# F-Fer/SLAM-Loop-Closing

Measured on AMD Instinct MI355X. Metric: Hamming distances/sec (256-bit ORB) for all-vs-all loop search, 1/2/4/8 GPUs, higher is better.
Workload: dtype u32

## Files before the change

include/lcm.h:

```cpp
#ifndef LCM_H_
#define LCM_H_

#include <stddef.h>
#include <stdint.h>

#ifdef __cplusplus
extern "C" {
#endif

#if defined(__GNUC__)
#define LCM_API __attribute__((visibility("default")))
#else
#define LCM_API
#endif

#define LCM_DESC_BYTES 32
#define LCM_DESC_WORDS 8
#define LCM_MAX_TRAIN_ROWS (1 << 22)

typedef enum lcm_status {
    LCM_OK = 0,
    LCM_ERR_INVALID_ARG = -1,
    LCM_ERR_NO_DEVICE = -2,
    LCM_ERR_HIP = -3,
// ... 362 lines not shown
                                          const int* query_frame_ids, int n_queries, int* ticket);
LCM_API int  lcm_group_query_collect_batch(lcm_group* g, int ticket, lcm_score* out_scores, size_t cap, size_t* n_out,
                                           size_t* offsets);
LCM_API int  lcm_group_online_stats_read(lcm_group* g, lcm_online_stats* out, int reset);
LCM_API int  lcm_group_detect_loops(lcm_group* g, int current_frame_id, const uint8_t* query, int nq, int n_keypoints,
                                    lcm_loop_candidate* out, int cap, int* n_out);
LCM_API int  lcm_merge_shard_scores(const lcm_score* const* shard_scores, const size_t* shard_counts, int world,
                                    const int32_t* ids, int n_frames, int min_gap,
                                    lcm_score* out, size_t cap, size_t* n_out, size_t* offsets);

LCM_API int  lcm_merge_shard_scores_device(lcm_handle* h, const void* d_gathered, const size_t* shard_counts, int world,
                                           const int32_t* ids, int n_frames, int min_gap,
                                           void* d_merged, size_t cap, size_t* n_out);

typedef enum lcm_tuning { LCM_TUNE_ITEM_SLOTS = 0, LCM_TUNE_ONLINE_SPLIT = 1, LCM_TUNE_PACKED = 2, LCM_TUNE_ONLINE_STREAMS = 3,
                          LCM_TUNE_PACKED_SCRATCH_MB = 4, LCM_TUNE_PAIR_UPLOAD_KERNEL = 5, LCM_TUNE_PAIR_HOST_FOLD = 6 } lcm_tuning;
LCM_API int  lcm_set_tuning(lcm_handle* h, int knob, int value);

LCM_API int  lcm_dev_alloc(lcm_handle* h, size_t bytes, void** d_ptr);
LCM_API int  lcm_dev_free(lcm_handle* h, void* d_ptr);
LCM_API int  lcm_dev_upload(lcm_handle* h, void* d_dst, const void* src, size_t bytes);
LCM_API int  lcm_dev_download(lcm_handle* h, void* dst, const void* d_src, size_t bytes);

#ifdef __cplusplus
}
#endif
#endif
```

slam-loop-closing_amd/capi.py:

```python
from __future__ import annotations

import ctypes as C
import os
from typing import Optional, Sequence, Tuple

import numpy as np

_HERE = os.path.dirname(os.path.abspath(__file__))
LIB_PATH = os.environ.get("LCM_LIB_PATH") or os.path.join(_HERE, "lib", "liblcm_hip.so")
DESC_BYTES = 32
SIFT_BYTES = 128
KEY_SHIFT = 22
TUNE_ITEM_SLOTS, TUNE_ONLINE_SPLIT, TUNE_PACKED, TUNE_ONLINE_STREAMS, TUNE_PACKED_SCRATCH_MB = 0, 1, 2, 3, 4
TUNE_PAIR_UPLOAD_KERNEL, TUNE_PAIR_HOST_FOLD = 5, 6


OK, ERR_INVALID_ARG, ERR_NO_DEVICE, ERR_HIP, ERR_CAPACITY, ERR_ORDER, ERR_NOT_FOUND, ERR_OOM = 0, -1, -2, -3, -4, -5, -6, -7


class LcmError(RuntimeError):
    def __init__(self, code: int, msg: str):
        super().__init__(f"lcm error {code}: {msg}")
        self.code = code


class Params(C.Structure):
    _fields_ = [("ratio", C.c_int32), ("dist_floor", C.c_int32), ("min_matches", C.c_int32),
                ("min_gap", C.c_int32), ("sim_threshold", C.c_double), ("cross_check", C.c_int32),
                ("reserved", C.c_int32)]
# ... 1534 lines not shown
```

slam-loop-closing_amd/csrc/lcm_api.cpp:

```cpp
#include "lcm_internal.h"

namespace lcm {
std::string& last_error() { static thread_local std::string e; return e; }
int fail(int code, const char* fmt, ...) {
    char buf[512];
    va_list ap;
    va_start(ap, fmt);
    vsnprintf(buf, sizeof buf, fmt, ap);
    va_end(ap);
    last_error() = buf;
    return code;
}
void set_last_error(const char* msg) { last_error() = msg ? msg : ""; }
}

namespace lcm {

int set_device(const lcm_handle* h) {
    HIP_TRY(hipSetDevice(h->device));
    return LCM_OK;
}

int wait_db(lcm_handle* h) {
    if (h->pending_copy) {
// ... 261 lines not shown
            if (value < 0 || value > 64) return fail(LCM_ERR_INVALID_ARG, "item slots must be 0 (automatic) .. 64");
            h->tune_item_slots = value; h->plan.key = 0; return LCM_OK;
        case LCM_TUNE_ONLINE_SPLIT:
            if (value != -1 && value != 0 && value != 1 && value != 2 && value != 4 && value != 16 && value != 32)
                return fail(LCM_ERR_INVALID_ARG, "online split must be -1 (automatic), 0 (off), 1, 2, 4 (rows per lane of a 256-thread workgroup), 16 or 32 (64 / 128 threads x 8 rows)");
            h->tune_online_split = value; return LCM_OK;
        case LCM_TUNE_ONLINE_STREAMS:
            if (value != 0 && value != 1) return fail(LCM_ERR_INVALID_ARG, "online streams must be 0 (the handle's stream) or 1 (one per query slot)");
            h->tune_online_streams = value; return LCM_OK;
        case LCM_TUNE_PAIR_UPLOAD_KERNEL:
            if (value != 0 && value != 1) return fail(LCM_ERR_INVALID_ARG, "pair upload must be 0 (hipMemcpyAsync) or 1 (kernel)");
            h->tune_pair_upload_kernel = value; return LCM_OK;
        case LCM_TUNE_PAIR_HOST_FOLD:
            if (value != 0 && value != 1) return fail(LCM_ERR_INVALID_ARG, "pair host fold must be 0 (device buffer + copy) or 1 (pinned host memory)");
            h->tune_pair_host_fold = value; return LCM_OK;
        case LCM_TUNE_PACKED_SCRATCH_MB:
            if (value < 1 || value > 65536) return fail(LCM_ERR_INVALID_ARG, "packed scratch must be 1 .. 65536 MiB per chunk");
            h->pk_scratch_cfg_words = h->pk_scratch_words = (size_t)value << 18; h->plan.key = 0; return LCM_OK;
        case LCM_TUNE_PACKED:
            if (value < -1 || value > 2) return fail(LCM_ERR_INVALID_ARG, "packed rows must be -1 (automatic), 0 (off), 1 (on) or 2 (on, 1536-row columns)");
            h->tune_packed = value; h->plan.key = 0; return LCM_OK;
        default: return fail(LCM_ERR_INVALID_ARG, "unknown tuning knob %d", knob);
    }
}


static int db_reserve_impl(lcm_handle* h, int n_frames, int max_desc) {
    if (!h || n_frames < 0 || max_desc < 0) return fail(LCM_ERR_INVALID_ARG, "bad argument");
    if (max_desc > MAX_FRAME_ROWS) return fail(LCM_ERR_CAPACITY, "a stored frame may hold at most %d rows (got %d)", MAX_FRAME_ROWS, max_desc);
    int rc = set_device(h); if (rc) return rc;
// ... 173 lines not shown


int lcm_loop_test(const lcm_params* p, const lcm_score* s, int n_query_kp, int n_train_kp, double* similarity) {
    if (similarity) *similarity = 0.0;
    if (!p || !s) return 0;
    const int den = std::min(n_query_kp, n_train_kp);
    if (den <= 0) return 0;
    const double sim = (double)s->good_count / (double)den;
    if (similarity) *similarity = sim;
    return (sim > p->sim_threshold) && ((long long)s->good_count >= (long long)p->min_matches);
}

int lcm_last_launch_info(const lcm_handle* hc, lcm_launch_info* info) {
    lcm_handle* h = const_cast<lcm_handle*>(hc);
    if (!h || !info) return fail(LCM_ERR_INVALID_ARG, "NULL argument");
    if (h->info_pending || h->aux_pending) { const int rc = set_device(h); if (rc) return rc; }
    if (h->info_pending) {
        HIP_TRY(hipEventSynchronize(h->ev_stop));
        float ms = 0.f;
        HIP_TRY(hipEventElapsedTime(&ms, h->ev_start, h->ev_stop));
        h->info.kernel_ms = ms;
        h->info.aux_kernel_ms = 0.0;
        h->info_pending = false;
        h->info.score_launches = 0; h->info.score_ms_sum = 0.0;
        if (h->info.route == LCM_ROUTE_PACKED) {
            double fold = 0.0, score = 0.0;
            for (size_t k = 0; k + 3 <= h->fold_ev_used && k + 3 <= h->fold_ev.size(); k += 3) {
                float f = 0.f;
                if (hipEventElapsedTime(&f, h->fold_ev[k], h->fold_ev[k + 1]) == hipSuccess) score += f; else (void)hipGetLastError();
                if (hipEventElapsedTime(&f, h->fold_ev[k + 1], h->fold_ev[k + 2]) == hipSuccess) fold += f; else (void)hipGetLastError();
                ++h->info.score_launches;
// ... 79 lines not shown
```

slam-loop-closing_amd/csrc/lcm_internal.h:

```cpp
#pragma once
#include "../../include/lcm.h"

#include <hip/hip_runtime.h>
#include <sys/stat.h>

#include <algorithm>
#include <cstdarg>
#include <cstdio>
#include <cstdlib>
#include <cstring>
#include <new>
#include <string>
#include <vector>

#include "lcm_kernels.h"
#include "lcm_l2_host.h"
#include "lcm_verify_host.h"

namespace lcm {
std::string& last_error();
int fail(int code, const char* fmt, ...) __attribute__((format(printf, 2, 3)));
void set_last_error(const char* msg);
}

// ... 110 lines not shown
    hipStream_t copy_stream = nullptr;
    hipStream_t stream2 = nullptr;
    hipEvent_t ev_fork = nullptr, ev_join = nullptr;
    hipEvent_t db_ready = nullptr;
    hipEvent_t ev_start = nullptr, ev_stop = nullptr;
    hipEvent_t ev_aux_start = nullptr, ev_aux_stop = nullptr;
    bool aux_pending = false;
    std::vector<hipEvent_t> fold_ev;
    size_t fold_ev_used = 0;
    int variant = 0;
    int tune_item_slots = 0;
    int tune_online_split = -1;
    int tune_pair_upload_kernel = 1;
    int tune_pair_host_fold = 1;
    int tune_online_streams = 1;
    size_t pk_scratch_cfg_words = (size_t)1 << 28;
    size_t pk_scratch_words = (size_t)1 << 28;
    bool pk_oom_retry = false;
    int tune_packed = -1;

    uint8_t* d_rows = nullptr;
    int32_t* d_counts = nullptr;
    int cap_frames = 0;
    int stride_rows = 0;
    std::vector<FrameMeta> frames;
    bool pending_copy = false;
    bool db_ready_recorded = false;

    uint8_t* h_stage[lcm::STAGE_BUFS] = {nullptr, nullptr};
    size_t h_stage_bytes = 0;
// ... 65 lines not shown
    struct PoseScratch {
        double* d_E = nullptr;        size_t d_E_n = 0;
        uint8_t* d_mask_in = nullptr; size_t d_mask_in_n = 0;
        double* d_cand = nullptr;     size_t d_cand_n = 0;
        lcm_pose_result* d_res = nullptr; size_t d_res_n = 0;
        uint8_t* d_mask = nullptr;    size_t d_mask_n = 0;
    } pose;
    struct LoScratch {
        int32_t* d_seeds = nullptr;   size_t d_seeds_n = 0;
        lcm_lo_info* d_info = nullptr; size_t d_info_n = 0;
        double* d_models = nullptr;   size_t d_models_n = 0;
        int32_t* d_seam = nullptr;    size_t d_seam_n = 0;
    } lo;
    lcm_launch_info info{};
    bool info_pending = false;
};


namespace {

template <typename T>
int ensure_dev(T*& p, size_t& have, size_t need, size_t slack_bytes = 0) {
    if (need <= have && p) return LCM_OK;
    if (p) HIP_TRY(hipFree(p));
    p = nullptr; have = 0;
    size_t n = std::max<size_t>(need, 16);
    HIP_TRY(hipMalloc((void**)&p, n * sizeof(T) + slack_bytes));
    have = n;
    return LCM_OK;
}
// ... 153 lines not shown
```

slam-loop-closing_amd/csrc/lcm_kernels.h:

```cpp
#pragma once
#include <hip/hip_runtime.h>
#include <stdint.h>

namespace lcm {

constexpr int KEY_SHIFT = 22;
constexpr uint32_t KEY_IDX_MASK = (1u << KEY_SHIFT) - 1;
constexpr int MAX_FUSED_QUERY_ROWS = 2048;
constexpr int MAX_QUERY_BATCH = 16;

struct WorkItem {
    uint32_t q_frame;
    uint32_t slot_begin;
    uint32_t n_slots;
    uint32_t out_offset;
};

struct PairItem {
    uint32_t q_row;
    uint32_t t_row;
    uint32_t nq_nt;
    uint32_t out_offset;
};

// ... 2 lines not shown
    const int32_t*  q_counts;
    uint32_t        q_stride_words;
    const uint32_t* db_rows;
    const int32_t*  db_counts;
    uint32_t        db_stride_words;
    const WorkItem* items;
    const PairItem* pair_items;
    void*           scores;
    uint32_t*       keys;
    uint32_t        keys_stride;
    uint32_t*       idx_sums;
    int32_t         ratio;
    int32_t         dist_floor;
    uint32_t        imp_chunks, imp_chunk_rows, imp_spi, imp_total;
    int32_t         imp_nq;
    const uint32_t* pk_vstart;
    const uint32_t* pk_qframe;
    const uint32_t* pk_elig;
    const uint32_t* pk_pairs;
    uint32_t*       pk_dist;
    uint32_t        pk_n;
    uint32_t        pk_col_rows;
    uint32_t        pk_stride;
    uint32_t        pk_slot0;
    uint32_t        imp_nbatch;
    uint32_t        bat_wg[MAX_QUERY_BATCH + 1];
    uint32_t        bat_pair[MAX_QUERY_BATCH + 1];
    int32_t         bat_nq[MAX_QUERY_BATCH];
    uint32_t        bat_elig[MAX_QUERY_BATCH];
};

hipError_t launch_score(const ScoreArgs& a, uint32_t n_items, int max_query_rows, bool write_keys, int variant,
                        hipStream_t st);
hipError_t launch_score_packed(const ScoreArgs& a, uint32_t n_items, bool argmin, hipStream_t st);

hipError_t launch_score_split(const ScoreArgs& a, uint32_t n_items, int qpt, hipStream_t st);
struct FinalizeArgs {
    const uint32_t* dist;
    uint32_t        padded_rows;
    int32_t         nq;
    const int32_t*  db_counts;
    uint32_t        slot_begin;
    void*           scores;
    int32_t         ratio, dist_floor;
    uint32_t        n_batch;
    uint32_t        bat_pair[MAX_QUERY_BATCH + 1];
    int32_t         bat_nq[MAX_QUERY_BATCH];
};
hipError_t launch_finalize(const FinalizeArgs& a, uint32_t n_pairs, hipStream_t st);

struct PairDesc {
    uint32_t first_item;
    uint32_t n_seg;
    uint32_t seg_rows;
// ... 283 lines not shown
```

slam-loop-closing_amd/csrc/lcm_kernels.hip:

```cpp
#include <hip/hip_runtime.h>
#include <stdint.h>

#include <algorithm>
#include <atomic>

#include "lcm_kernels.h"

#ifndef LCM_INNER_PRIO
#define LCM_INNER_PRIO 1
#endif

namespace lcm {

typedef const uint32_t __attribute__((address_space(4))) * sptr_t;
typedef const int32_t __attribute__((address_space(4))) * siptr_t;

__device__ __forceinline__ void fold2(uint32_t& best, const uint32_t (&q)[8], const uint32_t* s, uint32_t t0, uint32_t t1) {
#if LCM_INNER_PRIO
    uint32_t d0, d1, x0, x1;
    asm volatile(
        "v_xor_b32_e32 %3, %5, %21\n\tv_xor_b32_e32 %4, %13, %21\n\ts_setprio 3\n\t"
        "v_bcnt_u32_b32 %1, %3, 0\n\tv_bcnt_u32_b32 %2, %4, 0\n\ts_setprio 0\n\t"
        "v_xor_b32_e32 %3, %6, %22\n\tv_xor_b32_e32 %4, %14, %22\n\ts_setprio 3\n\t"
        "v_bcnt_u32_b32 %1, %3, %1\n\tv_bcnt_u32_b32 %2, %4, %2\n\ts_setprio 0\n\t"
// ... 149 lines not shown
        pair_nt = (int)(pi.nq_nt >> 12);
        pair_t_row = pi.t_row;
        q_word0 = (size_t)pi.q_row * 8;
    } else if (a.items) {
        it = a.items[blockIdx.x];
        nq = a.q_counts[it.q_frame];
        q_word0 = (size_t)it.q_frame * a.q_stride_words;
    } else {
        uint32_t b = blockIdx.x, qi = 0, total = a.imp_total, pair0 = 0;
        int rows = a.imp_nq;
        if (a.imp_nbatch) {
            while (qi + 1 < a.imp_nbatch && b >= a.bat_wg[qi + 1]) ++qi;
            b -= a.bat_wg[qi];
            total = a.bat_elig[qi]; pair0 = a.bat_pair[qi]; rows = a.bat_nq[qi];
        }
        const uint32_t c = b % a.imp_chunks, g = b / a.imp_chunks;
        it.q_frame = qi * a.imp_chunks + c;
        it.slot_begin = g * a.imp_spi;
        it.n_slots = min(a.imp_spi, total - it.slot_begin);
        it.out_offset = (pair0 + it.slot_begin) * a.imp_chunks + c;
        nq = min((int)a.imp_chunk_rows, rows - (int)(c * a.imp_chunk_rows));
        q_word0 = (size_t)it.q_frame * a.q_stride_words;
    }

    uint32_t q[QPT][8];
    auto valid = [&](int j) { return j * THREADS + tid < nq; };
    if (PACKED) {
        {
            uint32_t c = it.out_offset;
            const uint32_t v0 = it.q_frame * (uint32_t)(THREADS * QPT);
#pragma unroll 1
            for (int j = 0; j < QPT; ++j) {
                const uint32_t v = v0 + (uint32_t)(j * THREADS + tid);
                uint32_t meta = 0xFFFFFFFFu;
                if (j * THREADS + tid < nq) {
                    while (a.pk_vstart[c + 1] <= v) ++c;
                    meta = c;
// ... 381 lines not shown
    return hipGetLastError();
}

__global__ __launch_bounds__(256) void k_finalize_pairs(FinalizeArgs a, uint32_t n_pairs) {
    const int lane = threadIdx.x & 63;
    const uint32_t pair = blockIdx.x * 4u + (threadIdx.x >> 6);
    if (pair >= n_pairs) return;
    int nq = a.nq;
    uint32_t slot = a.slot_begin + pair;
    if (a.n_batch) {
        uint32_t b = 0;
        while (b + 1 < a.n_batch && pair >= a.bat_pair[b + 1]) ++b;
        nq = a.bat_nq[b];
        slot = pair - a.bat_pair[b];
    }
    const uint4* d = reinterpret_cast<const uint4*>(a.dist + (size_t)pair * a.padded_rows);
    uint32_t v[32];
#pragma unroll
    for (int i = 0; i < 8; ++i) {
        const int r0 = (i * 64 + lane) * 4;
        uint4 x = make_uint4(0xFFFFFFFFu, 0xFFFFFFFFu, 0xFFFFFFFFu, 0xFFFFFFFFu);
        if (r0 < nq) x = d[i * 64 + lane];
        v[4 * i + 0] = x.x;
        v[4 * i + 1] = r0 + 1 < nq ? x.y : 0xFFFFFFFFu;
        v[4 * i + 2] = r0 + 2 < nq ? x.z : 0xFFFFFFFFu;
        v[4 * i + 3] = r0 + 3 < nq ? x.w : 0xFFFFFFFFu;
    }
    uint32_t dmin = 0xFFFFFFFFu;
#pragma unroll
    for (int k = 0; k < 32; ++k) dmin = min(dmin, v[k]);
#pragma unroll
    for (int o = 32; o >= 1; o >>= 1) dmin = min(dmin, (uint32_t)__shfl_xor((int)dmin, o, 64));
    const uint32_t thr = max((uint32_t)a.ratio * dmin, (uint32_t)a.dist_floor);
    uint32_t cnt = 0;
#pragma unroll
    for (int k = 0; k < 32; ++k) cnt += (v[k] != 0xFFFFFFFFu && v[k] <= thr) ? 1u : 0u;
#pragma unroll
    for (int o = 32; o >= 1; o >>= 1) cnt += (uint32_t)__shfl_xor((int)cnt, o, 64);
    if (lane == 0) {
        const int nt = a.db_counts[slot];
        const bool empty = (nq <= 0) || (nt <= 0) || dmin == 0xFFFFFFFFu;
// ... 308 lines not shown
```

slam-loop-closing_amd/csrc/lcm_online.cpp:

```cpp
#include "lcm_internal.h"

static inline bool is_split(int qpt) { return qpt == 1 || qpt == 2 || qpt == 4 || qpt == 16 || qpt == 32; }
static inline int split_chunk_rows(int qpt) { return qpt == 16 ? 512 : qpt == 32 ? 1024 : 256 * qpt; }

static int pick_online_split(const lcm_handle* h, int max_nq, size_t pairs, bool batch) {
    if (h->variant != 0 || max_nq <= 512) return 0;
    if (h->tune_online_split >= 0) return h->tune_online_split;
    if (batch) return pairs < lcm::ONLINE_SPLIT_MAX_PAIRS ? 2 : 0;
    return pairs < 48 ? 1 : pairs < 4096 ? 2 : 0;
}

extern "C" {

static void account_prefix(lcm_handle* h, int nq, int n_elig) {
    uint64_t dist = 0, bytes = (uint64_t)nq * 32;
    for (int s = 0; s < n_elig; ++s) { dist += (uint64_t)nq * h->frames[s].n; bytes += (uint64_t)h->frames[s].n * 32 + 8; }
    h->info.pairs = (uint64_t)n_elig; h->info.distances = dist; h->info.algo_bytes = bytes;
}

static int enqueue_query(lcm_handle* h, QuerySlot& q, const uint32_t* d_q, int nq, int n_elig, hipStream_t S) {
    q.n_elig = n_elig; q.nq = nq; q.n_batch = 0;
    q.acc_pairs = q.acc_distances = q.acc_bytes = 0; q.acc_launches = 0; q.acc_queries = 1;
    if (n_elig <= 0) { HIP_TRY(hipEventRecord(q.done, S)); return LCM_OK; }
    int rc = wait_db(h); if (rc) return rc;
    if (h->params.cross_check) {
        rc = ensure_dev(q.d_scores, q.d_scores_n, (size_t)n_elig); if (rc) return rc;
        rc = ensure_pinned(q.h_scores, q.h_scores_n, (size_t)n_elig); if (rc) return rc;
        const uint32_t row0 = 0;
        HIP_TRY(hipEventRecord(q.k0, h->stream));
        rc = cross_score_prefixes(h, (const uint8_t*)d_q, &row0, &nq, &n_elig, 1, q.d_scores, nullptr); if (rc) return rc;
        HIP_TRY(hipEventRecord(q.k1, h->stream));
        q.acc_pairs = h->info.pairs; q.acc_distances = h->info.distances; q.acc_bytes = h->info.algo_bytes; q.acc_launches = h->info.launches;
        HIP_TRY(hipMemcpyAsync(q.h_scores, q.d_scores, sizeof(lcm_score) * (size_t)n_elig, hipMemcpyDeviceToHost, h->stream));
        HIP_TRY(hipEventRecord(q.done, h->stream));
        return LCM_OK;
    }
    if (h->variant >= 4) {
        return mfma_online(h, q, d_q, std::max(nq, 1), 1, &nq, &n_elig);
    }
    const int qpt = pick_online_split(h, nq, (size_t)n_elig, false);
    rc = ensure_dev(q.d_scores, q.d_scores_n, (size_t)n_elig); if (rc) return rc;
    rc = ensure_pinned(q.h_scores, q.h_scores_n, (size_t)n_elig); if (rc) return rc;
    lcm::ScoreArgs a{};
    a.q_rows = d_q; a.q_counts = nullptr; a.items = nullptr;
    a.db_rows = (const uint32_t*)h->d_rows; a.db_counts = h->d_counts; a.db_stride_words = (uint32_t)h->stride_rows * LCM_DESC_WORDS;
    a.ratio = h->params.ratio; a.dist_floor = h->params.dist_floor;
    a.imp_nq = nq; a.imp_total = (uint32_t)n_elig;
    HIP_TRY(hipEventRecord(h->ev_start, S));
    HIP_TRY(hipEventRecord(q.k0, S));
    if (is_split(qpt)) {
        const int chunk_rows = split_chunk_rows(qpt);
        const int n_chunks = (nq + chunk_rows - 1) / chunk_rows;
        const size_t n_items = (size_t)n_elig * n_chunks;
        rc = ensure_dev(q.d_dist, q.d_dist_n, n_items * chunk_rows); if (rc) return rc;
        a.q_stride_words = (uint32_t)chunk_rows * LCM_DESC_WORDS;
        a.imp_chunks = (uint32_t)n_chunks; a.imp_chunk_rows = (uint32_t)chunk_rows; a.imp_spi = 1;
        a.scores = nullptr ; a.keys = q.d_dist; a.keys_stride = (uint32_t)chunk_rows;
        hipError_t e = lcm::launch_score_split(a, (uint32_t)n_items, qpt, S);
        if (e != hipSuccess) return fail(LCM_ERR_HIP, "kernel launch failed: %s", hipGetErrorString(e));
        lcm::FinalizeArgs f{};
        f.dist = q.d_dist; f.padded_rows = (uint32_t)(n_chunks * chunk_rows); f.nq = nq;
        f.db_counts = h->d_counts; f.slot_begin = 0; f.scores = q.d_scores;
        f.ratio = h->params.ratio; f.dist_floor = h->params.dist_floor;
        e = lcm::launch_finalize(f, (uint32_t)n_elig, S);
        if (e != hipSuccess) return fail(LCM_ERR_HIP, "finalize launch failed: %s", hipGetErrorString(e));
        h->info.launches = 2; h->info.workgroups = (uint32_t)n_items; h->info.route = LCM_ROUTE_SPLIT;
    } else {
        const int spi = n_elig >= 8192 ? 4 : (n_elig >= 4096 ? 2 : 1);
        const uint32_t n_items = (uint32_t)((n_elig + spi - 1) / spi);
        a.q_stride_words = 0;
        a.imp_chunks = 1; a.imp_chunk_rows = (uint32_t)std::max(nq, 1); a.imp_spi = (uint32_t)spi;
        a.scores = q.d_scores; a.keys = nullptr; a.keys_stride = 0;
        hipError_t e = lcm::launch_score(a, n_items, nq, false, h->variant, S);
        if (e != hipSuccess) return fail(LCM_ERR_HIP, "kernel launch failed: %s", hipGetErrorString(e));
        h->info.launches = 1; h->info.workgroups = n_items; h->info.route = LCM_ROUTE_PLAIN;
    }
    HIP_TRY(hipEventRecord(h->ev_stop, S));
    HIP_TRY(hipEventRecord(q.k1, S));
    h->info_pending = true;
    account_prefix(h, nq, n_elig);
    q.acc_pairs = h->info.pairs; q.acc_distances = h->info.distances; q.acc_bytes = h->info.algo_bytes;
    q.acc_launches = h->info.launches; q.acc_queries = 1;
    HIP_TRY(hipMemcpyAsync(q.h_scores, q.d_scores, sizeof(lcm_score) * (size_t)n_elig, hipMemcpyDeviceToHost, S));
    HIP_TRY(hipEventRecord(q.done, S));
    return LCM_OK;
}

static int enqueue_batch(lcm_handle* h, QuerySlot& q, const uint32_t* d_q, int rows_per_query, int B, const int* nq, const int* elig, hipStream_t S) {
    size_t total = 0;
    int max_nq = 0;
    for (int b = 0; b < B; ++b) { total += (size_t)elig[b]; max_nq = std::max(max_nq, nq[b]); q.bat_elig[b] = elig[b]; }
    q.n_batch = B; q.n_elig = (int)total; q.nq = max_nq;
    q.acc_pairs = q.acc_distances = q.acc_bytes = 0; q.acc_launches = 0; q.acc_queries = (uint32_t)B;
    if (total == 0) { HIP_TRY(hipEventRecord(q.done, S)); return LCM_OK; }
    if (total > 0x7FFFFFFFull) return fail(LCM_ERR_CAPACITY, "more than 2^31 pairs in one batch");
    int rc = wait_db(h); if (rc) return rc;
    if (h->params.cross_check) {
        rc = ensure_dev(q.d_scores, q.d_scores_n, total); if (rc) return rc;
        rc = ensure_pinned(q.h_scores, q.h_scores_n, total); if (rc) return rc;
        uint32_t row0[lcm::MAX_QUERY_BATCH];
        for (int b = 0; b < B; ++b) row0[b] = (uint32_t)(b * rows_per_query);
        HIP_TRY(hipEventRecord(q.k0, h->stream));
        rc = cross_score_prefixes(h, (const uint8_t*)d_q, row0, nq, elig, B, q.d_scores, nullptr); if (rc) return rc;
        HIP_TRY(hipEventRecord(q.k1, h->stream));
        q.acc_pairs = h->info.pairs; q.acc_distances = h->info.distances; q.acc_bytes = h->info.algo_bytes; q.acc_launches = h->info.launches;
        HIP_TRY(hipMemcpyAsync(q.h_scores, q.d_scores, sizeof(lcm_score) * total, hipMemcpyDeviceToHost, h->stream));
        HIP_TRY(hipEventRecord(q.done, h->stream));
        return LCM_OK;
    }
    if (h->variant >= 4) return mfma_online(h, q, d_q, rows_per_query, B, nq, elig);
    const int qpt = pick_online_split(h, max_nq, total, true);
    rc = ensure_dev(q.d_scores, q.d_scores_n, total); if (rc) return rc;
    rc = ensure_pinned(q.h_scores, q.h_scores_n, total); if (rc) return rc;
    lcm::ScoreArgs a{};
    a.q_rows = d_q; a.q_counts = nullptr; a.items = nullptr;
    a.db_rows = (const uint32_t*)h->d_rows; a.db_counts = h->d_counts; a.db_stride_words = (uint32_t)h->stride_rows * LCM_DESC_WORDS;
    a.ratio = h->params.ratio; a.dist_floor = h->params.dist_floor;
    a.imp_nbatch = (uint32_t)B;
    const bool split = is_split(qpt);
    const int chunk_rows = split ? split_chunk_rows(qpt) : rows_per_query;
    const int n_chunks = split ? (max_nq + chunk_rows - 1) / chunk_rows : 1;
    if (rows_per_query % chunk_rows != 0 || n_chunks * chunk_rows > rows_per_query)
        return fail(LCM_ERR_INVALID_ARG, "batch staging pitch %d does not fit %d chunks of %d rows", rows_per_query, n_chunks, chunk_rows);
    const int spi = split ? 1 : (total >= 16384 ? 4 : (total >= 8192 ? 2 : 1));
    const uint32_t chunk_slots = (uint32_t)(rows_per_query / chunk_rows);
    a.q_stride_words = (uint32_t)chunk_rows * LCM_DESC_WORDS;
    a.imp_chunks = (uint32_t)n_chunks; a.imp_chunk_rows = (uint32_t)chunk_rows; a.imp_spi = (uint32_t)spi;
    uint32_t wg = 0, pair = 0;
    for (int b = 0; b < B; ++b) {
        a.bat_wg[b] = wg; a.bat_pair[b] = pair;
        a.bat_nq[b] = nq[b]; a.bat_elig[b] = (uint32_t)elig[b];
        wg += (uint32_t)((elig[b] + spi - 1) / spi) * (uint32_t)n_chunks;
        pair += (uint32_t)elig[b];
    }
    a.bat_wg[B] = wg; a.bat_pair[B] = pair;
    if ((uint32_t)n_chunks != chunk_slots) return fail(LCM_ERR_HIP, "internal: batch pitch %u != %d chunks", chunk_slots, n_chunks);
    HIP_TRY(hipEventRecord(h->ev_start, S));
    HIP_TRY(hipEventRecord(q.k0, S));
    if (split) {
        rc = ensure_dev(q.d_dist, q.d_dist_n, total * (size_t)n_chunks * chunk_rows); if (rc) return rc;
        a.scores = nullptr; a.keys = q.d_dist; a.keys_stride = (uint32_t)chunk_rows;
        hipError_t e = lcm::launch_score_split(a, wg, qpt, S);
        if (e != hipSuccess) return fail(LCM_ERR_HIP, "kernel launch failed: %s", hipGetErrorString(e));
        lcm::FinalizeArgs f{};
        f.dist = q.d_dist; f.padded_rows = (uint32_t)(n_chunks * chunk_rows); f.nq = 0;
        f.db_counts = h->d_counts; f.slot_begin = 0; f.scores = q.d_scores;
        f.ratio = h->params.ratio; f.dist_floor = h->params.dist_floor;
        f.n_batch = (uint32_t)B;
        for (int b = 0; b <= B; ++b) f.bat_pair[b] = a.bat_pair[b];
        for (int b = 0; b < B; ++b) f.bat_nq[b] = nq[b];
        e = lcm::launch_finalize(f, pair, S);
        if (e != hipSuccess) return fail(LCM_ERR_HIP, "finalize launch failed: %s", hipGetErrorString(e));
        h->info.launches = 2; h->info.route = LCM_ROUTE_SPLIT;
    } else {
        a.scores = q.d_scores; a.keys = nullptr; a.keys_stride = 0;
        hipError_t e = lcm::launch_score(a, wg, max_nq, false, h->variant >= 2 ? 0 : h->variant, S);
        if (e != hipSuccess) return fail(LCM_ERR_HIP, "kernel launch failed: %s", hipGetErrorString(e));
        h->info.launches = 1; h->info.route = LCM_ROUTE_PLAIN;
    }
    h->info.workgroups = wg;
    HIP_TRY(hipEventRecord(h->ev_stop, S));
    HIP_TRY(hipEventRecord(q.k1, S));
    h->info_pending = true;
    {
        uint64_t dist = 0, bytes = 0, prows = 0;
        int s = 0;
        std::vector<std::pair<int, int>> order((size_t)B);
        for (int b = 0; b < B; ++b) order[(size_t)b] = {elig[b], b};
        std::sort(order.begin(), order.end());
        for (auto [e, b] : order) {
            for (; s < e; ++s) prows += (uint64_t)h->frames[(size_t)s].n;
            dist += (uint64_t)nq[b] * prows;
            bytes += prows * 32 + (uint64_t)nq[b] * 32 + 8ull * (uint64_t)e;
        }
        h->info.pairs = total; h->info.distances = dist; h->info.algo_bytes = bytes;
        q.acc_pairs = total; q.acc_distances = dist; q.acc_bytes = bytes; q.acc_launches = h->info.launches;
    }
    HIP_TRY(hipMemcpyAsync(q.h_scores, q.d_scores, sizeof(lcm_score) * total, hipMemcpyDeviceToHost, S));
    HIP_TRY(hipEventRecord(q.done, S));
    return LCM_OK;
}

static int enqueue_big(lcm_handle* h, QuerySlot& q, const void* d_q, const int32_t* d_counts, int stride_rows, int B,
                       const int* nq, const int* ids, const int* elig) {
    size_t total = 0;
    int max_nq = 0;
    for (int b = 0; b < B; ++b) { total += (size_t)elig[b]; max_nq = std::max(max_nq, nq[b]); q.bat_elig[b] = elig[b]; }
    q.n_elig = (int)total; q.nq = max_nq;
    q.acc_pairs = q.acc_distances = q.acc_bytes = 0; q.acc_launches = 0; q.acc_queries = (uint32_t)B;
    if (total == 0) { HIP_TRY(hipEventRecord(q.done, h->stream)); return LCM_OK; }
    if (total > 0x7FFFFFFFull) return fail(LCM_ERR_CAPACITY, "more than 2^31 pairs in one batch");
    int rc = ensure_dev(q.d_scores, q.d_scores_n, total); if (rc) return rc;
    rc = ensure_pinned(q.h_scores, q.h_scores_n, total); if (rc) return rc;
// ... 6 lines not shown
    q.acc_pairs = h->info.pairs; q.acc_distances = h->info.distances; q.acc_bytes = h->info.algo_bytes; q.acc_launches = h->info.launches;
    HIP_TRY(hipMemcpyAsync(q.h_scores, q.d_scores, sizeof(lcm_score) * total, hipMemcpyDeviceToHost, h->stream));
    HIP_TRY(hipEventRecord(q.done, h->stream));
    return LCM_OK;
}

static int upload_counts(lcm_handle* h, QuerySlot& q, const int* nq, int B) {
    int rc = ensure_pinned(q.h_meta, q.h_meta_bytes, sizeof(int32_t) * (size_t)lcm::MAX_QUERY_BATCH); if (rc) return rc;
    rc = ensure_dev(q.d_meta, q.d_meta_bytes, sizeof(int32_t) * (size_t)lcm::MAX_QUERY_BATCH); if (rc) return rc;
    memcpy(q.h_meta, nq, sizeof(int32_t) * (size_t)B);
    HIP_TRY(hipMemcpyAsync(q.d_meta, q.h_meta, sizeof(int32_t) * (size_t)B, hipMemcpyHostToDevice, h->stream));
    return LCM_OK;
}

static void fold_online_stats(lcm_handle* h, QuerySlot& q) {
    if (q.acc_launches) {
        float ms = 0.f;
        if (hipEventElapsedTime(&ms, q.k0, q.k1) == hipSuccess) h->online.kernel_ms += ms; else (void)hipGetLastError();
    }
    h->online.launches += q.acc_launches; h->online.queries += q.acc_queries;
    h->online.pairs += q.acc_pairs; h->online.distances += q.acc_distances; h->online.algo_bytes += q.acc_bytes;
    q.acc_launches = 0; q.acc_queries = 0; q.acc_pairs = q.acc_distances = q.acc_bytes = 0;
}

static int find_slot(const lcm_handle* h, int frame_id) {
    int lo = 0, hi = (int)h->frames.size();
    while (lo < hi) { int mid = (lo + hi) / 2; if (h->frames[mid].id < frame_id) lo = mid + 1; else hi = mid; }
    return (lo < (int)h->frames.size() && h->frames[lo].id == frame_id) ? lo : -1;
}

static int acquire_query_slot(lcm_handle* h, int* ticket) {
    for (int i = 0; i < QUERY_SLOTS; ++i)
        if (!h->qslots[i].busy) {
            if (!h->qslots[i].done) HIP_TRY(hipEventCreateWithFlags(&h->qslots[i].done, hipEventDisableTiming));
// ... 17 lines not shown
    return LCM_OK;
}

static int query_submit_impl(lcm_handle* h, const uint8_t* query, int nq, int query_frame_id, int* ticket) {
    if (!h || nq < 0 || !ticket || (nq > 0 && !query)) return fail(LCM_ERR_INVALID_ARG, "bad argument");
    *ticket = -1;
    if (nq > 65535) return fail(LCM_ERR_CAPACITY, "a frame may hold at most 65535 rows (got %d)", nq);
    const bool big = nq > lcm::MAX_FUSED_QUERY_ROWS;
    int rc = set_device(h); if (rc) return rc;
    int t = -1;
    rc = acquire_query_slot(h, &t); if (rc) return rc;
    QuerySlot& q = h->qslots[t];
    q.query_id = query_frame_id;
    const int n_elig = eligible_prefix(h, query_frame_id, h->params.min_gap);
    const int rows_up = h->params.cross_check ? padded_rows(nq) + ROW_PAD : nq;
    const size_t bytes = (size_t)std::max(rows_up, 1) * LCM_DESC_BYTES;
    rc = ensure_pinned(q.h_query, q.h_query_bytes, bytes); if (rc) return rc;
    rc = ensure_dev(q.d_query, q.d_query_bytes, bytes, ARENA_SLACK); if (rc) return rc;
    hipStream_t S = h->stream;
    if (!big) { rc = pick_stream(h, q, &S); if (rc) return rc; }
    if (nq > 0 && n_elig > 0) {
        memcpy(q.h_query, query, (size_t)nq * LCM_DESC_BYTES);
        for (int r = nq; r < rows_up; ++r) memcpy(q.h_query + (size_t)r * LCM_DESC_BYTES, query + (size_t)(nq - 1) * LCM_DESC_BYTES, LCM_DESC_BYTES);
        HIP_TRY(hipMemcpyAsync(q.d_query, q.h_query, (size_t)rows_up * LCM_DESC_BYTES, hipMemcpyHostToDevice, S));
    }
    if (big) {
        q.n_batch = 0;
        rc = upload_counts(h, q, &nq, 1); if (rc) return rc;
        rc = enqueue_big(h, q, q.d_query, reinterpret_cast<const int32_t*>(q.d_meta), rows_up, 1, &nq, &query_frame_id, &n_elig); if (rc) return rc;
    } else {
        rc = enqueue_query(h, q, (const uint32_t*)q.d_query, nq, n_elig, S); if (rc) return rc;
    }
    q.busy = true;
    q.db_generation = h->db_generation;
    *ticket = t;
    return LCM_OK;
}

static int query_collect_impl(lcm_handle* h, int ticket, lcm_score* out_scores, int32_t* out_frame_ids, int cap, int* n_out) {
// ... 33 lines not shown
    }
    int rc = set_device(h); if (rc) return rc;
    int t = -1;
    rc = acquire_query_slot(h, &t); if (rc) return rc;
    QuerySlot& q = h->qslots[t];
    q.query_id = query_frame_ids[0];
    int elig[lcm::MAX_QUERY_BATCH];
    size_t total = 0;
    for (int b = 0; b < n_queries; ++b) { elig[b] = eligible_prefix(h, query_frame_ids[b], h->params.min_gap); total += (size_t)elig[b]; }
    int pitch = std::max(max_nq, 1);
    {
        const int qpt = pick_online_split(h, max_nq, total, true);
        if (is_split(qpt)) pitch = round_up(max_nq, split_chunk_rows(qpt));
    }
    if (h->params.cross_check) pitch = padded_rows(std::max(max_nq, 1)) + 2 * ROW_PAD;
    const size_t bytes = (size_t)pitch * (size_t)n_queries * LCM_DESC_BYTES;
    rc = ensure_pinned(q.h_query, q.h_query_bytes, bytes); if (rc) return rc;
    rc = ensure_dev(q.d_query, q.d_query_bytes, bytes, ARENA_SLACK); if (rc) return rc;
    const bool big = max_nq > lcm::MAX_FUSED_QUERY_ROWS;
    hipStream_t S = h->stream;
    if (!big) { rc = pick_stream(h, q, &S); if (rc) return rc; }
    if (total > 0) {
        for (int b = 0; b < n_queries; ++b)
            if (nq[b] > 0) {
                uint8_t* dst = q.h_query + (size_t)b * pitch * LCM_DESC_BYTES;
                memcpy(dst, queries[b], (size_t)nq[b] * LCM_DESC_BYTES);
                if (h->params.cross_check)
                    for (int r = nq[b]; r < padded_rows(nq[b]) + ROW_PAD; ++r) memcpy(dst + (size_t)r * LCM_DESC_BYTES, queries[b] + (size_t)(nq[b] - 1) * LCM_DESC_BYTES, LCM_DESC_BYTES);
            }
        HIP_TRY(hipMemcpyAsync(q.d_query, q.h_query, bytes, hipMemcpyHostToDevice, S));
    }
    if (big) {
        q.n_batch = n_queries;
        rc = upload_counts(h, q, nq, n_queries); if (rc) return rc;
        rc = enqueue_big(h, q, q.d_query, reinterpret_cast<const int32_t*>(q.d_meta), pitch, n_queries, nq, query_frame_ids, elig); if (rc) return rc;
    } else {
        rc = enqueue_batch(h, q, (const uint32_t*)q.d_query, pitch, n_queries, nq, elig, S); if (rc) return rc;
    }
    q.busy = true;
    q.db_generation = h->db_generation;
    *ticket = t;
    return LCM_OK;
}

static int query_collect_batch_impl(lcm_handle* h, int ticket, lcm_score* out_scores, size_t cap, size_t* n_out, size_t* offsets) {
// ... 112 lines not shown
```

Before: 4311 billion.

## Cut online query overheads: kernel upload, host-mapped records, train segmentation

Small online queries now upload through a copy kernel instead of hipMemcpyAsync, and finalize/score kernels write records straight into pinned host memory, which removes the device-to-host copy. Small split launches can also divide train rows into segments so there are more workgroups, and finalize takes the min across segments. The change drops the shared ev_start/ev_stop events and the wait_db call on side streams, and reads timing from per-slot events instead. The risks are slower zero-copy writes over PCIe, extra finalize reads, and ordering issues when a side stream skips wait_db.

Result: no change. 4317 billion, median of 6 (+0.1%).

```diff
diff --git a/include/lcm.h b/include/lcm.h
--- a/include/lcm.h
+++ b/include/lcm.h
@@ -400,7 +400,8 @@
                                            void* d_merged, size_t cap, size_t* n_out);
 
 typedef enum lcm_tuning { LCM_TUNE_ITEM_SLOTS = 0, LCM_TUNE_ONLINE_SPLIT = 1, LCM_TUNE_PACKED = 2, LCM_TUNE_ONLINE_STREAMS = 3,
-                          LCM_TUNE_PACKED_SCRATCH_MB = 4, LCM_TUNE_PAIR_UPLOAD_KERNEL = 5, LCM_TUNE_PAIR_HOST_FOLD = 6 } lcm_tuning;
+                          LCM_TUNE_PACKED_SCRATCH_MB = 4, LCM_TUNE_PAIR_UPLOAD_KERNEL = 5, LCM_TUNE_PAIR_HOST_FOLD = 6,
+                          LCM_TUNE_ONLINE_UPLOAD_KERNEL = 7, LCM_TUNE_ONLINE_HOST_RECORDS = 8, LCM_TUNE_ONLINE_TRAIN_SEGS = 9 } lcm_tuning;
 LCM_API int  lcm_set_tuning(lcm_handle* h, int knob, int value);
 
 LCM_API int  lcm_dev_alloc(lcm_handle* h, size_t bytes, void** d_ptr);
diff --git a/slam-loop-closing_amd/capi.py b/slam-loop-closing_amd/capi.py
--- a/slam-loop-closing_amd/capi.py
+++ b/slam-loop-closing_amd/capi.py
@@ -13,6 +13,7 @@
 KEY_SHIFT = 22
 TUNE_ITEM_SLOTS, TUNE_ONLINE_SPLIT, TUNE_PACKED, TUNE_ONLINE_STREAMS, TUNE_PACKED_SCRATCH_MB = 0, 1, 2, 3, 4
 TUNE_PAIR_UPLOAD_KERNEL, TUNE_PAIR_HOST_FOLD = 5, 6
+TUNE_ONLINE_UPLOAD_KERNEL, TUNE_ONLINE_HOST_RECORDS, TUNE_ONLINE_TRAIN_SEGS = 7, 8, 9
 
 
 OK, ERR_INVALID_ARG, ERR_NO_DEVICE, ERR_HIP, ERR_CAPACITY, ERR_ORDER, ERR_NOT_FOUND, ERR_OOM = 0, -1, -2, -3, -4, -5, -6, -7
diff --git a/slam-loop-closing_amd/csrc/lcm_api.cpp b/slam-loop-closing_amd/csrc/lcm_api.cpp
--- a/slam-loop-closing_amd/csrc/lcm_api.cpp
+++ b/slam-loop-closing_amd/csrc/lcm_api.cpp
@@ -299,6 +299,15 @@
         case LCM_TUNE_PAIR_HOST_FOLD:
             if (value != 0 && value != 1) return fail(LCM_ERR_INVALID_ARG, "pair host fold must be 0 (device buffer + copy) or 1 (pinned host memory)");
             h->tune_pair_host_fold = value; return LCM_OK;
+        case LCM_TUNE_ONLINE_UPLOAD_KERNEL:
+            if (value != 0 && value != 1) return fail(LCM_ERR_INVALID_ARG, "online upload must be 0 (hipMemcpyAsync) or 1 (kernel)");
+            h->tune_online_upload_kernel = value; return LCM_OK;
+        case LCM_TUNE_ONLINE_HOST_RECORDS:
+            if (value != 0 && value != 1) return fail(LCM_ERR_INVALID_ARG, "online host records must be 0 (device buffer + copy) or 1 (pinned host memory)");
+            h->tune_online_host_records = value; return LCM_OK;
+        case LCM_TUNE_ONLINE_TRAIN_SEGS:
+            if (value < -1 || value > 16) return fail(LCM_ERR_INVALID_ARG, "online train segments must be -1 (automatic), 0 / 1 (none) or 2 .. 16");
+            h->tune_online_train_segs = value; return LCM_OK;
         case LCM_TUNE_PACKED_SCRATCH_MB:
             if (value < 1 || value > 65536) return fail(LCM_ERR_INVALID_ARG, "packed scratch must be 1 .. 65536 MiB per chunk");
             h->pk_scratch_cfg_words = h->pk_scratch_words = (size_t)value << 18; h->plan.key = 0; return LCM_OK;
@@ -502,7 +511,18 @@
 int lcm_last_launch_info(const lcm_handle* hc, lcm_launch_info* info) {
     lcm_handle* h = const_cast<lcm_handle*>(hc);
     if (!h || !info) return fail(LCM_ERR_INVALID_ARG, "NULL argument");
-    if (h->info_pending || h->aux_pending) { const int rc = set_device(h); if (rc) return rc; }
+    if (h->info_pending || h->aux_pending || h->info_slot >= 0) { const int rc = set_device(h); if (rc) return rc; }
+    if (h->info_slot >= 0 && !h->info_pending) {
+        const QuerySlot& q = h->qslots[h->info_slot];
+        HIP_TRY(hipEventSynchronize(q.k1));
+        float ms = 0.f;
+        HIP_TRY(hipEventElapsedTime(&ms, q.k0, q.k1));
+        h->info.kernel_ms = ms;
+        h->info.aux_kernel_ms = 0.0;
+        h->info.score_launches = 0; h->info.score_ms_sum = 0.0;
+        h->info.launches_in_flight = 1;
+    }
+    h->info_slot = -1;
     if (h->info_pending) {
         HIP_TRY(hipEventSynchronize(h->ev_stop));
         float ms = 0.f;
diff --git a/slam-loop-closing_amd/csrc/lcm_internal.h b/slam-loop-closing_amd/csrc/lcm_internal.h
--- a/slam-loop-closing_amd/csrc/lcm_internal.h
+++ b/slam-loop-closing_amd/csrc/lcm_internal.h
@@ -148,6 +148,9 @@
     int tune_pair_upload_kernel = 1;
     int tune_pair_host_fold = 1;
     int tune_online_streams = 1;
+    int tune_online_upload_kernel = 1;
+    int tune_online_host_records = 1;
+    int tune_online_train_segs = -1;
     size_t pk_scratch_cfg_words = (size_t)1 << 28;
     size_t pk_scratch_words = (size_t)1 << 28;
     bool pk_oom_retry = false;
@@ -243,6 +246,7 @@
     } lo;
     lcm_launch_info info{};
     bool info_pending = false;
+    int info_slot = -1;
 };
 
 
diff --git a/slam-loop-closing_amd/csrc/lcm_kernels.h b/slam-loop-closing_amd/csrc/lcm_kernels.h
--- a/slam-loop-closing_amd/csrc/lcm_kernels.h
+++ b/slam-loop-closing_amd/csrc/lcm_kernels.h
@@ -40,6 +40,7 @@
     int32_t         dist_floor;
     uint32_t        imp_chunks, imp_chunk_rows, imp_spi, imp_total;
     int32_t         imp_nq;
+    uint32_t        imp_tseg, imp_tseg_rows;
     const uint32_t* pk_vstart;
     const uint32_t* pk_qframe;
     const uint32_t* pk_elig;
@@ -64,6 +65,7 @@
 struct FinalizeArgs {
     const uint32_t* dist;
     uint32_t        padded_rows;
+    uint32_t        n_seg;
     int32_t         nq;
     const int32_t*  db_counts;
     uint32_t        slot_begin;
diff --git a/slam-loop-closing_amd/csrc/lcm_kernels.hip b/slam-loop-closing_amd/csrc/lcm_kernels.hip
--- a/slam-loop-closing_amd/csrc/lcm_kernels.hip
+++ b/slam-loop-closing_amd/csrc/lcm_kernels.hip
@@ -187,13 +187,21 @@
             b -= a.bat_wg[qi];
             total = a.bat_elig[qi]; pair0 = a.bat_pair[qi]; rows = a.bat_nq[qi];
         }
-        const uint32_t c = b % a.imp_chunks, g = b / a.imp_chunks;
+        const uint32_t c = b % a.imp_chunks;
+        uint32_t g = b / a.imp_chunks, seg = 0;
+        const uint32_t n_seg = (WRITE_KEYS && !ARGMIN) ? max(a.imp_tseg, 1u) : 1u;
+        if (n_seg > 1) { seg = g % n_seg; g /= n_seg; }
         it.q_frame = qi * a.imp_chunks + c;
         it.slot_begin = g * a.imp_spi;
         it.n_slots = min(a.imp_spi, total - it.slot_begin);
-        it.out_offset = (pair0 + it.slot_begin) * a.imp_chunks + c;
+        it.out_offset = ((pair0 + it.slot_begin) * n_seg + seg) * a.imp_chunks + c;
         nq = min((int)a.imp_chunk_rows, rows - (int)(c * a.imp_chunk_rows));
         q_word0 = (size_t)it.q_frame * a.q_stride_words;
+        if (n_seg > 1) {
+            const int seg0 = (int)(seg * a.imp_tseg_rows);
+            pair_nt = max(0, min((int)a.imp_tseg_rows, ((siptr_t)a.db_counts)[it.slot_begin] - seg0));
+            pair_t_row = it.slot_begin * (a.db_stride_words / 8u) + (uint32_t)seg0;
+        }
     }
 
     uint32_t q[QPT][8];
@@ -605,17 +613,29 @@
         nq = a.bat_nq[b];
         slot = pair - a.bat_pair[b];
     }
-    const uint4* d = reinterpret_cast<const uint4*>(a.dist + (size_t)pair * a.padded_rows);
+    const uint32_t n_seg = max(a.n_seg, 1u);
+    const uint4* d = reinterpret_cast<const uint4*>(a.dist + (size_t)pair * n_seg * a.padded_rows);
     uint32_t v[32];
+#pragma unroll
+    for (int k = 0; k < 32; ++k) v[k] = 0xFFFFFFFFu;
+    for (uint32_t s = 0; s < n_seg; ++s) {
+        const uint4* ds = d + (size_t)s * (a.padded_rows / 4);
+#pragma unroll
+        for (int i = 0; i < 8; ++i) {
+            const int r0 = (i * 64 + lane) * 4;
+            if (r0 < nq) {
+                const uint4 x = ds[i * 64 + lane];
+                v[4 * i + 0] = min(v[4 * i + 0], x.x); v[4 * i + 1] = min(v[4 * i + 1], x.y);
+                v[4 * i + 2] = min(v[4 * i + 2], x.z); v[4 * i + 3] = min(v[4 * i + 3], x.w);
+            }
+        }
+    }
 #pragma unroll
     for (int i = 0; i < 8; ++i) {
         const int r0 = (i * 64 + lane) * 4;
-        uint4 x = make_uint4(0xFFFFFFFFu, 0xFFFFFFFFu, 0xFFFFFFFFu, 0xFFFFFFFFu);
-        if (r0 < nq) x = d[i * 64 + lane];
-        v[4 * i + 0] = x.x;
-        v[4 * i + 1] = r0 + 1 < nq ? x.y : 0xFFFFFFFFu;
-        v[4 * i + 2] = r0 + 2 < nq ? x.z : 0xFFFFFFFFu;
-        v[4 * i + 3] = r0 + 3 < nq ? x.w : 0xFFFFFFFFu;
+        if (r0 + 1 >= nq) v[4 * i + 1] = 0xFFFFFFFFu;
+        if (r0 + 2 >= nq) v[4 * i + 2] = 0xFFFFFFFFu;
+        if (r0 + 3 >= nq) v[4 * i + 3] = 0xFFFFFFFFu;
     }
     uint32_t dmin = 0xFFFFFFFFu;
 #pragma unroll
diff --git a/slam-loop-closing_amd/csrc/lcm_online.cpp b/slam-loop-closing_amd/csrc/lcm_online.cpp
--- a/slam-loop-closing_amd/csrc/lcm_online.cpp
+++ b/slam-loop-closing_amd/csrc/lcm_online.cpp
@@ -10,6 +10,41 @@
     return pairs < 48 ? 1 : pairs < 4096 ? 2 : 0;
 }
 
+static int pick_train_segs(const lcm_handle* h, size_t wgs, int n_slots, int* seg_rows) {
+    *seg_rows = 0;
+    if (h->tune_online_train_segs == 0 || h->tune_online_train_segs == 1 || wgs == 0) return 1;
+    if ((size_t)h->cap_frames * (size_t)h->stride_rows >= 0xFFFFFFFFull) return 1;
+    int want = h->tune_online_train_segs > 1 ? h->tune_online_train_segs : (int)std::min<size_t>(16, 2048 / wgs);
+    if (want <= 1) return 1;
+    int max_nt = 0;
+    for (int s2 = 0; s2 < n_slots; ++s2) max_nt = std::max(max_nt, h->frames[(size_t)s2].n);
+    const int min_rows = h->tune_online_train_segs > 1 ? 16 : 64;
+    const int rows = std::max(round_up((max_nt + want - 1) / want, 16), min_rows);
+    const int n_seg = (max_nt + rows - 1) / rows;
+    if (n_seg <= 1) return 1;
+    *seg_rows = rows;
+    return n_seg;
+}
+
+constexpr size_t ONLINE_UPLOAD_KERNEL_MAX_BYTES = (size_t)1 << 20;
+static inline size_t round16(size_t v) { return (v + 15) & ~(size_t)15; }
+
+static int upload_query(lcm_handle* h, QuerySlot& q, size_t bytes, bool by_kernel, hipStream_t S) {
+    if (by_kernel && h->tune_online_upload_kernel && bytes <= ONLINE_UPLOAD_KERNEL_MAX_BYTES) {
+        if (round16(bytes) > q.h_query_bytes || round16(bytes) > q.d_query_bytes) return fail(LCM_ERR_HIP, "internal: query staging smaller than the upload");
+        const hipError_t e = lcm::launch_upload(q.d_query, q.h_query, bytes, S);
+        if (e != hipSuccess) return fail(LCM_ERR_HIP, "upload kernel launch failed: %s", hipGetErrorString(e));
+        return LCM_OK;
+    }
+    HIP_TRY(hipMemcpyAsync(q.d_query, q.h_query, bytes, hipMemcpyHostToDevice, S));
+    return LCM_OK;
+}
+
+static void info_from_slot(lcm_handle* h, const QuerySlot& q) {
+    h->info_pending = false;
+    h->info_slot = (int)(&q - h->qslots);
+}
+
 extern "C" {
 
 static void account_prefix(lcm_handle* h, int nq, int n_elig) {
@@ -22,7 +57,7 @@
     q.n_elig = n_elig; q.nq = nq; q.n_batch = 0;
     q.acc_pairs = q.acc_distances = q.acc_bytes = 0; q.acc_launches = 0; q.acc_queries = 1;
     if (n_elig <= 0) { HIP_TRY(hipEventRecord(q.done, S)); return LCM_OK; }
-    int rc = wait_db(h); if (rc) return rc;
+    int rc = S == h->stream ? wait_db(h) : LCM_OK; if (rc) return rc;
     if (h->params.cross_check) {
         rc = ensure_dev(q.d_scores, q.d_scores_n, (size_t)n_elig); if (rc) return rc;
         rc = ensure_pinned(q.h_scores, q.h_scores_n, (size_t)n_elig); if (rc) return rc;
@@ -39,28 +74,32 @@
         return mfma_online(h, q, d_q, std::max(nq, 1), 1, &nq, &n_elig);
     }
     const int qpt = pick_online_split(h, nq, (size_t)n_elig, false);
-    rc = ensure_dev(q.d_scores, q.d_scores_n, (size_t)n_elig); if (rc) return rc;
+    const bool host_rec = h->tune_online_host_records != 0;
+    if (!host_rec) { rc = ensure_dev(q.d_scores, q.d_scores_n, (size_t)n_elig); if (rc) return rc; }
     rc = ensure_pinned(q.h_scores, q.h_scores_n, (size_t)n_elig); if (rc) return rc;
+    lcm_score* const rec = host_rec ? q.h_scores : q.d_scores;
     lcm::ScoreArgs a{};
     a.q_rows = d_q; a.q_counts = nullptr; a.items = nullptr;
     a.db_rows = (const uint32_t*)h->d_rows; a.db_counts = h->d_counts; a.db_stride_words = (uint32_t)h->stride_rows * LCM_DESC_WORDS;
     a.ratio = h->params.ratio; a.dist_floor = h->params.dist_floor;
     a.imp_nq = nq; a.imp_total = (uint32_t)n_elig;
-    HIP_TRY(hipEventRecord(h->ev_start, S));
     HIP_TRY(hipEventRecord(q.k0, S));
     if (is_split(qpt)) {
         const int chunk_rows = split_chunk_rows(qpt);
         const int n_chunks = (nq + chunk_rows - 1) / chunk_rows;
-        const size_t n_items = (size_t)n_elig * n_chunks;
+        int seg_rows = 0;
+        const int n_seg = pick_train_segs(h, (size_t)n_elig * n_chunks, n_elig, &seg_rows);
+        const size_t n_items = (size_t)n_elig * n_chunks * n_seg;
         rc = ensure_dev(q.d_dist, q.d_dist_n, n_items * chunk_rows); if (rc) return rc;
         a.q_stride_words = (uint32_t)chunk_rows * LCM_DESC_WORDS;
         a.imp_chunks = (uint32_t)n_chunks; a.imp_chunk_rows = (uint32_t)chunk_rows; a.imp_spi = 1;
+        a.imp_tseg = (uint32_t)n_seg; a.imp_tseg_rows = (uint32_t)seg_rows;
         a.scores = nullptr ; a.keys = q.d_dist; a.keys_stride = (uint32_t)chunk_rows;
         hipError_t e = lcm::launch_score_split(a, (uint32_t)n_items, qpt, S);
         if (e != hipSuccess) return fail(LCM_ERR_HIP, "kernel launch failed: %s", hipGetErrorString(e));
         lcm::FinalizeArgs f{};
-        f.dist = q.d_dist; f.padded_rows = (uint32_t)(n_chunks * chunk_rows); f.nq = nq;
-        f.db_counts = h->d_counts; f.slot_begin = 0; f.scores = q.d_scores;
+        f.dist = q.d_dist; f.padded_rows = (uint32_t)(n_chunks * chunk_rows); f.nq = nq; f.n_seg = (uint32_t)n_seg;
+        f.db_counts = h->d_counts; f.slot_begin = 0; f.scores = rec;
         f.ratio = h->params.ratio; f.dist_floor = h->params.dist_floor;
         e = lcm::launch_finalize(f, (uint32_t)n_elig, S);
         if (e != hipSuccess) return fail(LCM_ERR_HIP, "finalize launch failed: %s", hipGetErrorString(e));
@@ -70,18 +109,17 @@
         const uint32_t n_items = (uint32_t)((n_elig + spi - 1) / spi);
         a.q_stride_words = 0;
         a.imp_chunks = 1; a.imp_chunk_rows = (uint32_t)std::max(nq, 1); a.imp_spi = (uint32_t)spi;
-        a.scores = q.d_scores; a.keys = nullptr; a.keys_stride = 0;
+        a.scores = rec; a.keys = nullptr; a.keys_stride = 0;
         hipError_t e = lcm::launch_score(a, n_items, nq, false, h->variant, S);
         if (e != hipSuccess) return fail(LCM_ERR_HIP, "kernel launch failed: %s", hipGetErrorString(e));
         h->info.launches = 1; h->info.workgroups = n_items; h->info.route = LCM_ROUTE_PLAIN;
     }
-    HIP_TRY(hipEventRecord(h->ev_stop, S));
     HIP_TRY(hipEventRecord(q.k1, S));
-    h->info_pending = true;
+    info_from_slot(h, q);
     account_prefix(h, nq, n_elig);
     q.acc_pairs = h->info.pairs; q.acc_distances = h->info.distances; q.acc_bytes = h->info.algo_bytes;
     q.acc_launches = h->info.launches; q.acc_queries = 1;
-    HIP_TRY(hipMemcpyAsync(q.h_scores, q.d_scores, sizeof(lcm_score) * (size_t)n_elig, hipMemcpyDeviceToHost, S));
+    if (!host_rec) HIP_TRY(hipMemcpyAsync(q.h_scores, q.d_scores, sizeof(lcm_score) * (size_t)n_elig, hipMemcpyDeviceToHost, S));
     HIP_TRY(hipEventRecord(q.done, S));
     return LCM_OK;
 }
@@ -94,7 +132,7 @@
     q.acc_pairs = q.acc_distances = q.acc_bytes = 0; q.acc_launches = 0; q.acc_queries = (uint32_t)B;
     if (total == 0) { HIP_TRY(hipEventRecord(q.done, S)); return LCM_OK; }
     if (total > 0x7FFFFFFFull) return fail(LCM_ERR_CAPACITY, "more than 2^31 pairs in one batch");
-    int rc = wait_db(h); if (rc) return rc;
+    int rc = S == h->stream ? wait_db(h) : LCM_OK; if (rc) return rc;
     if (h->params.cross_check) {
         rc = ensure_dev(q.d_scores, q.d_scores_n, total); if (rc) return rc;
         rc = ensure_pinned(q.h_scores, q.h_scores_n, total); if (rc) return rc;
@@ -110,8 +148,10 @@
     }
     if (h->variant >= 4) return mfma_online(h, q, d_q, rows_per_query, B, nq, elig);
     const int qpt = pick_online_split(h, max_nq, total, true);
-    rc = ensure_dev(q.d_scores, q.d_scores_n, total); if (rc) return rc;
+    const bool host_rec = h->tune_online_host_records != 0;
+    if (!host_rec) { rc = ensure_dev(q.d_scores, q.d_scores_n, total); if (rc) return rc; }
     rc = ensure_pinned(q.h_scores, q.h_scores_n, total); if (rc) return rc;
+    lcm_score* const rec = host_rec ? q.h_scores : q.d_scores;
     lcm::ScoreArgs a{};
     a.q_rows = d_q; a.q_counts = nullptr; a.items = nullptr;
     a.db_rows = (const uint32_t*)h->d_rows; a.db_counts = h->d_counts; a.db_stride_words = (uint32_t)h->stride_rows * LCM_DESC_WORDS;
@@ -126,25 +166,27 @@
     const uint32_t chunk_slots = (uint32_t)(rows_per_query / chunk_rows);
     a.q_stride_words = (uint32_t)chunk_rows * LCM_DESC_WORDS;
     a.imp_chunks = (uint32_t)n_chunks; a.imp_chunk_rows = (uint32_t)chunk_rows; a.imp_spi = (uint32_t)spi;
+    int seg_rows = 0, n_seg = 1;
+    if (split) n_seg = pick_train_segs(h, total * (size_t)n_chunks, *std::max_element(elig, elig + B), &seg_rows);
+    a.imp_tseg = (uint32_t)n_seg; a.imp_tseg_rows = (uint32_t)seg_rows;
     uint32_t wg = 0, pair = 0;
     for (int b = 0; b < B; ++b) {
         a.bat_wg[b] = wg; a.bat_pair[b] = pair;
         a.bat_nq[b] = nq[b]; a.bat_elig[b] = (uint32_t)elig[b];
-        wg += (uint32_t)((elig[b] + spi - 1) / spi) * (uint32_t)n_chunks;
+        wg += (uint32_t)((elig[b] + spi - 1) / spi) * (uint32_t)n_chunks * (uint32_t)n_seg;
         pair += (uint32_t)elig[b];
     }
     a.bat_wg[B] = wg; a.bat_pair[B] = pair;
     if ((uint32_t)n_chunks != chunk_slots) return fail(LCM_ERR_HIP, "internal: batch pitch %u != %d chunks", chunk_slots, n_chunks);
-    HIP_TRY(hipEventRecord(h->ev_start, S));
     HIP_TRY(hipEventRecord(q.k0, S));
     if (split) {
-        rc = ensure_dev(q.d_dist, q.d_dist_n, total * (size_t)n_chunks * chunk_rows); if (rc) return rc;
+        rc = ensure_dev(q.d_dist, q.d_dist_n, total * (size_t)n_seg * (size_t)n_chunks * chunk_rows); if (rc) return rc;
         a.scores = nullptr; a.keys = q.d_dist; a.keys_stride = (uint32_t)chunk_rows;
         hipError_t e = lcm::launch_score_split(a, wg, qpt, S);
         if (e != hipSuccess) return fail(LCM_ERR_HIP, "kernel launch failed: %s", hipGetErrorString(e));
         lcm::FinalizeArgs f{};
-        f.dist = q.d_dist; f.padded_rows = (uint32_t)(n_chunks * chunk_rows); f.nq = 0;
-        f.db_counts = h->d_counts; f.slot_begin = 0; f.scores = q.d_scores;
+        f.dist = q.d_dist; f.padded_rows = (uint32_t)(n_chunks * chunk_rows); f.nq = 0; f.n_seg = (uint32_t)n_seg;
+        f.db_counts = h->d_counts; f.slot_begin = 0; f.scores = rec;
         f.ratio = h->params.ratio; f.dist_floor = h->params.dist_floor;
         f.n_batch = (uint32_t)B;
         for (int b = 0; b <= B; ++b) f.bat_pair[b] = a.bat_pair[b];
@@ -153,15 +195,14 @@
         if (e != hipSuccess) return fail(LCM_ERR_HIP, "finalize launch failed: %s", hipGetErrorString(e));
         h->info.launches = 2; h->info.route = LCM_ROUTE_SPLIT;
     } else {
-        a.scores = q.d_scores; a.keys = nullptr; a.keys_stride = 0;
+        a.scores = rec; a.keys = nullptr; a.keys_stride = 0;
         hipError_t e = lcm::launch_score(a, wg, max_nq, false, h->variant >= 2 ? 0 : h->variant, S);
         if (e != hipSuccess) return fail(LCM_ERR_HIP, "kernel launch failed: %s", hipGetErrorString(e));
         h->info.launches = 1; h->info.route = LCM_ROUTE_PLAIN;
     }
     h->info.workgroups = wg;
-    HIP_TRY(hipEventRecord(h->ev_stop, S));
     HIP_TRY(hipEventRecord(q.k1, S));
-    h->info_pending = true;
+    info_from_slot(h, q);
     {
         uint64_t dist = 0, bytes = 0, prows = 0;
         int s = 0;
@@ -176,7 +217,7 @@
         h->info.pairs = total; h->info.distances = dist; h->info.algo_bytes = bytes;
         q.acc_pairs = total; q.acc_distances = dist; q.acc_bytes = bytes; q.acc_launches = h->info.launches;
     }
-    HIP_TRY(hipMemcpyAsync(q.h_scores, q.d_scores, sizeof(lcm_score) * total, hipMemcpyDeviceToHost, S));
+    if (!host_rec) HIP_TRY(hipMemcpyAsync(q.h_scores, q.d_scores, sizeof(lcm_score) * total, hipMemcpyDeviceToHost, S));
     HIP_TRY(hipEventRecord(q.done, S));
     return LCM_OK;
 }
@@ -213,10 +254,18 @@
 }
 
 static void fold_online_stats(lcm_handle* h, QuerySlot& q) {
+    const bool is_info = h->info_slot == (int)(&q - h->qslots) && !h->info_pending;
     if (q.acc_launches) {
         float ms = 0.f;
-        if (hipEventElapsedTime(&ms, q.k0, q.k1) == hipSuccess) h->online.kernel_ms += ms; else (void)hipGetLastError();
-    }
+        if (hipEventElapsedTime(&ms, q.k0, q.k1) == hipSuccess) {
+            h->online.kernel_ms += ms;
+            if (is_info) {
+                h->info.kernel_ms = ms; h->info.aux_kernel_ms = 0.0;
+                h->info.score_launches = 0; h->info.score_ms_sum = 0.0; h->info.launches_in_flight = 1;
+            }
+        } else (void)hipGetLastError();
+    }
+    if (is_info) h->info_slot = -1;
     h->online.launches += q.acc_launches; h->online.queries += q.acc_queries;
     h->online.pairs += q.acc_pairs; h->online.distances += q.acc_distances; h->online.algo_bytes += q.acc_bytes;
     q.acc_launches = 0; q.acc_queries = 0; q.acc_pairs = q.acc_distances = q.acc_bytes = 0;
@@ -264,15 +313,16 @@
     q.query_id = query_frame_id;
     const int n_elig = eligible_prefix(h, query_frame_id, h->params.min_gap);
     const int rows_up = h->params.cross_check ? padded_rows(nq) + ROW_PAD : nq;
-    const size_t bytes = (size_t)std::max(rows_up, 1) * LCM_DESC_BYTES;
+    const size_t bytes = round16((size_t)std::max(rows_up, 1) * LCM_DESC_BYTES);
     rc = ensure_pinned(q.h_query, q.h_query_bytes, bytes); if (rc) return rc;
     rc = ensure_dev(q.d_query, q.d_query_bytes, bytes, ARENA_SLACK); if (rc) return rc;
     hipStream_t S = h->stream;
     if (!big) { rc = pick_stream(h, q, &S); if (rc) return rc; }
+    const bool up_by_kernel = !big && !h->params.cross_check && h->variant < 4;
     if (nq > 0 && n_elig > 0) {
         memcpy(q.h_query, query, (size_t)nq * LCM_DESC_BYTES);
         for (int r = nq; r < rows_up; ++r) memcpy(q.h_query + (size_t)r * LCM_DESC_BYTES, query + (size_t)(nq - 1) * LCM_DESC_BYTES, LCM_DESC_BYTES);
-        HIP_TRY(hipMemcpyAsync(q.d_query, q.h_query, (size_t)rows_up * LCM_DESC_BYTES, hipMemcpyHostToDevice, S));
+        rc = upload_query(h, q, (size_t)rows_up * LCM_DESC_BYTES, up_by_kernel, S); if (rc) return rc;
     }
     if (big) {
         q.n_batch = 0;
@@ -336,7 +386,7 @@
         if (is_split(qpt)) pitch = round_up(max_nq, split_chunk_rows(qpt));
     }
     if (h->params.cross_check) pitch = padded_rows(std::max(max_nq, 1)) + 2 * ROW_PAD;
-    const size_t bytes = (size_t)pitch * (size_t)n_queries * LCM_DESC_BYTES;
+    const size_t bytes = round16((size_t)pitch * (size_t)n_queries * LCM_DESC_BYTES);
     rc = ensure_pinned(q.h_query, q.h_query_bytes, bytes); if (rc) return rc;
     rc = ensure_dev(q.d_query, q.d_query_bytes, bytes, ARENA_SLACK); if (rc) return rc;
     const bool big = max_nq > lcm::MAX_FUSED_QUERY_ROWS;
@@ -350,7 +400,7 @@
                 if (h->params.cross_check)
                     for (int r = nq[b]; r < padded_rows(nq[b]) + ROW_PAD; ++r) memcpy(dst + (size_t)r * LCM_DESC_BYTES, queries[b] + (size_t)(nq[b] - 1) * LCM_DESC_BYTES, LCM_DESC_BYTES);
             }
-        HIP_TRY(hipMemcpyAsync(q.d_query, q.h_query, bytes, hipMemcpyHostToDevice, S));
+        rc = upload_query(h, q, bytes, !big && !h->params.cross_check && h->variant < 4, S); if (rc) return rc;
     }
     if (big) {
         q.n_batch = n_queries;
```
